# henriChevreux/distillation_trajectories

Measured on AMD Instinct MI355X. Metric: trajectory-timesteps/sec (B×T U-Net fwd) at 16×16 T=50, higher is better.
Workload: dtype f32 (fp32-accurate; convolutions: exact 3-plane bf16 operand split on bf16 MFMA with fp32 accumulate, or native fp32 MFMA, chosen per layer)

## Files before the change

### distillation_trajectories_amd/_hip.py

```python
import ctypes
import os
from ctypes import (POINTER, c_char_p, c_double, c_float, c_int, c_int32, c_int64, c_longlong, c_size_t, c_uint8,
                    c_void_p)

_LIB = None
LIB_PATH = os.path.join(os.path.dirname(os.path.abspath(__file__)), "csrc", "libdt_hip.so")

COND_NONE, COND_ZERO, COND_ONE = 0, 1, 2
RULE_ENGINE, RULE_PSAMPLE, RULE_MANAGER = 0, 1, 2
PREC_FP32, PREC_SPLIT_BF16, PREC_AUTO = 0, 1, 2
KIND_FP32 = 0
KIND_NAMES = {KIND_FP32: "fp32", 1: "split-bf16", 3: "split-bf16-strip", 4: "split-bf16-strip32", 5: "split-bf16-stripk"}
BT_COUNT, GT_COUNT, N_BLOCKS = 16, 9, 8
ABI_VERSION = 5


class HipLibraryError(RuntimeError):
    pass


class UNetDesc(ctypes.Structure):
    _fields_ = [("channels", c_int32), ("dims", c_int32 * 4), ("temb_dim", c_int32)]


SIGNATURES = {
    "dt_abi_version": (c_int, []),
    "dt_status_string": (c_char_p, [c_int]),
    "dt_unet_create": (c_int, [POINTER(UNetDesc), POINTER(c_void_p), POINTER(c_void_p), c_void_p, POINTER(c_void_p)]),
    "dt_unet_destroy": (None, [c_void_p]),
    "dt_unet_time_bias_stride": (c_int, [c_void_p]),
    "dt_unet_time_bias": (c_int, [c_void_p, c_void_p, c_void_p, c_void_p, c_int, c_void_p, c_void_p]),
    "dt_unet_workspace_bytes": (c_size_t, [c_void_p, c_int, c_int, c_int]),
    "dt_unet_forward": (c_int, [c_void_p, c_void_p, c_int, c_int, c_int, c_int, c_void_p, c_int, c_void_p,
                                c_void_p, c_size_t, c_void_p]),
    "dt_unet_autotune": (c_int, [c_void_p, c_int, c_int, c_int, c_void_p, c_size_t, c_void_p]),
    "dt_unet_conv_choice": (c_int, [c_void_p, c_int, c_int, c_int, c_int, c_int, POINTER(c_int), POINTER(c_int),
                                    POINTER(c_int), POINTER(c_int), POINTER(c_int)]),
    "dt_unet_set_conv_choice": (c_int, [c_void_p] + [c_int] * 10),
    "dt_unet_declare_shape": (c_int, [c_void_p] + [c_int] * 5),
    "dt_unet_set_precision": (c_int, [c_void_p, c_int]),
    "dt_unet_set_head_fusion": (c_int, [c_void_p, c_int]),
    "dt_unet_set_fused": (c_int, [c_void_p, c_int]),
    "dt_unet_fused_active": (c_int, [c_void_p, c_int, c_int]),
    "dt_unet_time_conv": (c_int, [c_void_p, c_int, c_int, c_int, c_int, c_int, c_int, c_int, c_int, c_int, c_int, c_int,
                                  c_void_p, c_size_t, c_void_p, POINTER(c_float), POINTER(c_double)]),
# ... 94 lines not shown
```

### distillation_trajectories_amd/csrc/build.py

```python
import os
import shutil
import subprocess
import sys

HERE = os.path.dirname(os.path.abspath(__file__))
SOURCES = ["dt_conv.hip", "dt_conv_bf16.hip", "dt_conv_strip.hip", "dt_layers.hip", "dt_update.hip", "dt_metrics.hip", "dt_fused.hip", "dt_unet.hip"]
HEADERS = ["dt_internal.h", "dt_conv_epilogue.h", "dt_update_math.h", "dt_fused.h", os.path.join("..", "..", "include", "dt_hip.h"),
           os.path.join("..", "..", "include", "dt_hip_noise.h")]
LIB = os.path.join(HERE, "libdt_hip.so")
ARCH = "gfx950"


def hipcc_path():
    for cand in (os.environ.get("HIPCC"), "/opt/rocm/bin/hipcc", shutil.which("hipcc")):
        if cand and os.path.exists(cand):
            return cand
    raise RuntimeError("hipcc not found (looked at $HIPCC, /opt/rocm/bin/hipcc, PATH)")


OBJ_DIR = os.path.join(HERE, "_build")
FLAGS = [f"--offload-arch={ARCH}", "-O3", "-std=c++17", "-fPIC", "-Wall", "-Wno-unused-function"]


def _newer(target, deps):
    if not os.path.exists(target):
        return True
    t = os.path.getmtime(target)
    return any(os.path.getmtime(d) > t for d in deps)


def is_stale():
    deps = [os.path.join(HERE, f) for f in SOURCES + HEADERS] + [os.path.abspath(__file__)]
    return _newer(LIB, deps)


TOOLS_MARK = os.path.join(OBJ_DIR, "tools_build")


def build(force=False, verbose=False, tools=False):
# ... 79 lines not shown
```

### distillation_trajectories_amd/csrc/dt_conv.hip

```cpp
#include "dt_conv_epilogue.h"

namespace dt {

template <int BM, int BN>
__global__ __launch_bounds__(256, 4) void conv_gemm_kernel(const ConvParams p) {
  constexpr int WN = 2;
  constexpr int MI = BM / 64, NI = BN / 64;
  constexpr int A_PER = BM / 64, B_PER = BN / 64;
  constexpr int STAGE = (BM + BN) * 16;
  constexpr int LDS_FLOATS = 2 * STAGE > epilogue_stage_floats<BN>() ? 2 * STAGE : epilogue_stage_floats<BN>();
  __shared__ __attribute__((aligned(16))) float lds[LDS_FLOATS];

  const int tid = threadIdx.x, lane = tid & 63, wave = tid >> 6;
  const int wm = wave / WN, wn = wave % WN;
  const int half = lane >> 5, l31 = lane & 31;
  const int m0 = blockIdx.x * BM, n0 = blockIdx.y * BN;
  const int HW = p.H * p.W;
  const int CC = p.cin_p >> 4;

  int a_off[A_PER], a_off2[A_PER], a_y[A_PER], a_x[A_PER];
  bool a_ok[A_PER];
  int a_lds[A_PER];
#pragma unroll
  for (int j = 0; j < A_PER; ++j) {
// ... 69 lines not shown
#pragma unroll
        for (int i = 0; i < 4; ++i)
#pragma unroll
          for (int mi = 0; mi < MI; ++mi)
#pragma unroll
            for (int ni = 0; ni < NI; ++ni) {
              acc[mi][ni] = __builtin_amdgcn_mfma_f32_32x32x2f32(fa[mi][i], fb[ni][i], acc[mi][ni], 0, 0, 0);
            }
      }
    }
    if (more) {
      float *A = lds + ((it + 1) & 1) * STAGE, *B = A + BM * 16;
#pragma unroll
      for (int j = 0; j < A_PER; ++j) *reinterpret_cast<f32x4 *>(A + a_lds[j]) = ra[j];
#pragma unroll
      for (int j = 0; j < B_PER; ++j) *reinterpret_cast<f32x4 *>(B + (tid + j * 256) * 4) = rb[j];
    }
    __syncthreads();
  }

  conv_epilogue<MI, NI>(p, acc, lds, m0, n0, wm, wn, half, l31);
}

int launch_splitk_epilogue(const ConvParams &p, hipStream_t s);

int launch_conv(const ConvParams &p, hipStream_t s) {
  if (!p.in || !p.w || !p.scale || !p.shift || !p.out) return DT_E_NULL;
  if (p.cin_p % 16 || p.cout_p % 16 || p.n_p % kNPad || p.M <= 0) return DT_E_SHAPE;
  if ((long long)p.M * p.cin_p >= (1ll << 31) || (long long)p.M * p.cout_p * (p.n_dup > 1 ? p.n_dup : 1) >= (1ll << 31)) return DT_E_SHAPE;
  if (const int st = conv_admissible(p)) return st;
  const bool tall_m = p.bm == 128, wide_n = p.bn == 128;
  dim3 grid((p.M + p.bm - 1) / p.bm, p.n_p / p.bn, p.splits);
  const double flops = 2.0 * p.M * (double)p.cout_real * ((double)p.cin_real * p.ksize * p.ksize + (p.in2 ? p.cin2_real : 0));
  if (is_strip(p.kind)) {
    ProfileScope prof(p.kind == KIND_STRIPK ? (tall_m ? KC_CONVS_K128x64 : (wide_n ? KC_CONVS_K64x128 : KC_CONVS_K64x64)) : p.bm == 256 ? KC_CONVS_256x64 : tall_m ? (wide_n ? KC_CONVS_128x128 : KC_CONVS_128x64) : (wide_n ? KC_CONVS_64x128 : KC_CONVS_64x64),
                      flops, 4.0 * p.M * ((double)p.cin_real + p.cout_real), s);
    const int st = launch_conv_strip(p, s);
    if (st) return st;
  } else if (p.kind == KIND_BF16) {
    ProfileScope prof(tall_m ? (wide_n ? KC_CONVB_128x128 : KC_CONVB_128x64) : (wide_n ? KC_CONVB_64x128 : KC_CONVB_64x64),
                      flops, 4.0 * p.M * ((double)p.cin_real + p.cout_real), s);
    const int st = launch_conv_bf16x6(p, p.bm, p.bn, s);
    if (st) return st;
  } else {
    ProfileScope prof(tall_m ? (wide_n ? KC_CONV_128x128 : KC_CONV_128x64) : (wide_n ? KC_CONV_64x128 : KC_CONV_64x64),
                      flops, 4.0 * p.M * ((double)p.cin_real + p.cout_real), s);
    if (tall_m && wide_n) conv_gemm_kernel<128, 128><<<grid, 256, 0, s>>>(p);
    else if (tall_m) conv_gemm_kernel<128, 64><<<grid, 256, 0, s>>>(p);
    else if (wide_n) conv_gemm_kernel<64, 128><<<grid, 256, 0, s>>>(p);
    else conv_gemm_kernel<64, 64><<<grid, 256, 0, s>>>(p);
    DT_LAUNCH_CHECK();
  }
  if (p.splits > 1) return launch_splitk_epilogue(p, s);
  return DT_OK;
}


int strip_kc(int kind, int bm, int bn) { return kind == KIND_STRIPK ? (bm == 64 && bn == 64 ? 4 : 2) : (kind == KIND_STRIP2 ? 2 : 1); }

size_t strip_lds_bytes(int W, int bm, int bn, int kind) {
  const int kc = strip_kc(kind, bm, bn);
  const int R = bm + 2 * strip_halo(W, bm);
  const size_t loop = (size_t)kc * ((size_t)3 * (((R + 7) & ~7) + 8) * 16 + (kind == KIND_STRIPK ? 0 : (size_t)2 * 3 * bn * 16)) * sizeof(__bf16);
  const size_t stage = (size_t)(bm == 256 || (kind == KIND_STRIPK && bn == 64) ? 128 : 64) * (bn + 4) * sizeof(float);
  return loop > stage ? loop : stage;
}

bool strip_reaches(int W) { return W + 1 <= 64 && strip_lds_bytes(W, 64, 64, KIND_STRIP) <= strip_lds_limit(KIND_STRIP); }

static bool kind_has_tile(int kind, int bm, int bn) {
  if (kind < KIND_FP32 || kind > KIND_STRIPK || kind == 2) return false;
  if ((bm != 64 && bm != 128 && !(bm == 256 && bn == 64 && is_strip(kind))) || (bn != 64 && bn != 128)) return false;
  return !(kind == KIND_STRIPK && (bm > 128 || (bm == 128 && bn == 128)));
}

bool conv_choice_valid(const ConvChoice &c, int slot, int n_p) {
  if (!kind_has_tile(c.kind, c.bm, c.bn) || n_p % c.bn) return false;
  if (c.splits < 1 || c.splits > 9 || c.splits == 5 || c.splits == 6 || c.splits == 7) return false;
  return !c.fuse || (slot == 2 && c.splits == 1);
}

static ConvChoice heuristic_choice(int M, int n_p, int taps) {
  ConvChoice c{};
  c.bn = n_p % 128 == 0 ? 128 : 64;
  const long long blocks128 = (long long)((M + 127) / 128) * (n_p / c.bn);
  c.bm = blocks128 >= 512 ? 128 : 64;
  const long long blocks = (long long)((M + c.bm - 1) / c.bm) * (n_p / c.bn);
  c.splits = 1;
  if (taps == 9 && M <= kSplitMaxRows && blocks < 384) c.splits = blocks * 3 >= 384 ? 3 : 9;
  c.fuse = c.splits == 1;
  return c;
}

ConvChoice resolve_conv_choice(const ConvLayer &L, const ConvChoice *req, int precision) {
  ConvChoice c = req ? *req : heuristic_choice(L.M, L.n_p, L.splittable ? L.taps : 1);
  const int cc = L.cin_p >> 4;
  if (!req) {
    c.kind = precision == DT_PREC_FP32 ? KIND_FP32 : KIND_BF16;
    if (c.kind == KIND_BF16 && L.taps == 9 && strip_reaches(L.W)) {
      c.kind = KIND_STRIP;
      c.splits = c.splits == 9 ? (cc % 8 == 0 ? 8 : (cc % 4 == 0 ? 4 : 1)) : (c.splits == 3 ? (cc % 4 == 0 ? 4 : (cc % 2 == 0 ? 2 : 1)) : 1);
    }
  }
  if (c.kind == 2) c.kind = KIND_BF16;
  if (is_strip(c.kind) && (L.taps != 9 || !strip_reaches(L.W))) c.kind = KIND_BF16;
  if (c.kind == KIND_STRIPK && (c.bm > 128 || (c.bm == 128 && c.bn == 128))) c.kind = KIND_STRIP2;
  if (c.bm == 256 && !is_strip(c.kind)) c.bm = 128;
  if (!L.splittable) c.splits = 1;
  if (is_strip(c.kind) ? !chunks_fit(cc, pack_chunks(L.cin_p), c.splits * strip_kc(c.kind, c.bm, c.bn)) : (L.taps * cc) % c.splits != 0)
    c.splits = 1;
  c.fuse = L.foldable && c.fuse && c.splits == 1;
  return c;
}

int conv_admissible(const ConvParams &p) {
  const int cc = p.cin_p >> 4;
  if (!kind_has_tile(p.kind, p.bm, p.bn) || p.n_p % p.bn) return DT_E_ARG;
  if (p.splits < 1 || (p.splits > 1 && !p.slab)) return DT_E_ARG;
  if (p.ccw < cc || (p.in2 && p.ccw2 < (p.cin2_p >> 4))) return DT_E_ARG;
  if (p.in2 && (p.splits != 1 || !p.w2 || !p.bias2 || p.cin2_p % 16)) return DT_E_ARG;
  if (!is_strip(p.kind)) return (p.tap_hi - p.tap_lo) * cc % p.splits ? DT_E_ARG : DT_OK;
  const int kc = strip_kc(p.kind, p.bm, p.bn);
  if (p.ksize != 3 || p.tap_lo != 0 || p.tap_hi != 9 || !chunks_fit(cc, p.ccw, p.splits * kc)) return DT_E_ARG;
  if (kc == 4 && p.W + 1 > 32) return DT_E_SHAPE;
  if (p.in2 && !chunks_fit(p.cin2_p >> 4, p.ccw2, kc)) return DT_E_ARG;
  if (p.W + 1 > 64) return DT_E_SHAPE;
  return strip_lds_bytes(p.W, p.bm, p.bn, p.kind) <= strip_lds_limit(p.kind) ? DT_OK : DT_E_SHAPE;
}

template <int S>
__device__ inline float4 splitk_finish(const ConvParams &p, unsigned m, int n, size_t slab_stride) {
  const size_t o = (size_t)m * p.cout_p + n;
  float4 a;
  if (S > 0) {
    float4 part[S > 0 ? S : 1];
#pragma unroll
    for (int z = 0; z < S; ++z) part[z] = *reinterpret_cast<const float4 *>(p.slab + z * slab_stride + o);
    a = part[0];
#pragma unroll
    for (int z = 1; z < S; ++z) { a.x += part[z].x; a.y += part[z].y; a.z += part[z].z; a.w += part[z].w; }
  } else {
    a = *reinterpret_cast<const float4 *>(p.slab + o);
    for (int z = 1; z < p.splits; ++z) {
      const float4 b = *reinterpret_cast<const float4 *>(p.slab + z * slab_stride + o);
      a.x += b.x; a.y += b.y; a.z += b.z; a.w += b.w;
    }
  }
  const float4 sc = *reinterpret_cast<const float4 *>(p.scale + n), sh = *reinterpret_cast<const float4 *>(p.shift + n);
  float4 v = make_float4(a.x * sc.x + sh.x, a.y * sc.y + sh.y, a.z * sc.z + sh.z, a.w * sc.w + sh.w);
  if (p.relu) { v.x = fmaxf(v.x, 0.f); v.y = fmaxf(v.y, 0.f); v.z = fmaxf(v.z, 0.f); v.w = fmaxf(v.w, 0.f); }
  if (p.tb) {
    const float4 t = *reinterpret_cast<const float4 *>(p.tb + (size_t)(m / (unsigned)p.m_per_tb) * p.tb_stride + n);
    v.x += t.x; v.y += t.y; v.z += t.z; v.w += t.w;
// ... 137 lines not shown
```

### distillation_trajectories_amd/csrc/dt_conv_epilogue.h

```cpp
#pragma once
#include "dt_internal.h"

namespace dt {

typedef float f32x16 __attribute__((ext_vector_type(16)));
typedef float f32x4 __attribute__((ext_vector_type(4)));

typedef __bf16 bf16x8 __attribute__((ext_vector_type(8)));
typedef __bf16 bf16x2 __attribute__((ext_vector_type(2)));
typedef unsigned u32x4 __attribute__((ext_vector_type(4)));

__device__ inline float bf16_to_f32(__bf16 v) { return (float)v; }

__device__ inline void split8(const f32x4 lo, const f32x4 hi, bf16x8 &p1, bf16x8 &p2, bf16x8 &p3) {
#pragma unroll
  for (int i = 0; i < 8; ++i) {
    const float a = i < 4 ? lo[i] : hi[i - 4];
    const __bf16 a1 = (__bf16)a;
    const float r1 = a - (float)a1;
    const __bf16 a2 = (__bf16)r1;
    const float r2 = r1 - (float)a2;
    p1[i] = a1; p2[i] = a2; p3[i] = (__bf16)r2;
  }
}

template <int BN, int WM = 2>
constexpr int epilogue_stage_floats() { return WM * 32 * (BN + 4); }

template <int MI, int NI, int WM = 2, int WK = 1>
__device__ inline void conv_epilogue(const ConvParams &p, f32x16 (&acc)[MI][NI], float *stage, int m0, int n0, int wm, int wn,
                                     int half, int l31, int wk = 0) {
  constexpr int BN = NI * 32 * (4 / (WM * WK)), P = BN + 4, C4 = BN / 4, U = WM * C4 / 8;
  constexpr int COPY = WM * 32 * P;
  const int tid = threadIdx.x;
  const int HW = p.H * p.W;
  const bool pow2 = (p.W & (p.W - 1)) == 0 && (HW & (HW - 1)) == 0;
  const int w_sh = 31 - __builtin_clz(p.W), hw_sh = 31 - __builtin_clz(HW);
  auto div_hw = [&](int m) { return pow2 ? m >> hw_sh : m / HW; };
  auto div_w = [&](int r) { return pow2 ? r >> w_sh : r / p.W; };
  const bool slab_mode = p.splits > 1;
  const size_t slab_stride = (size_t)p.M * p.cout_p;
  const int c4 = tid % C4, row0 = tid / C4;
  const int n = n0 + c4 * 4;
  const bool n_ok = n < p.cout_p;
  const int nn = n_ok ? n : 0;
  auto unit = [&](int k) __attribute__((always_inline)) {
    const float *src = stage + (row0 + k * (256 / C4)) * P + c4 * 4;
    f32x4 v = *reinterpret_cast<const f32x4 *>(src);
#pragma unroll
    for (int c = 1; c < WK; ++c) v += *reinterpret_cast<const f32x4 *>(src + c * COPY);
    return v;
  };
  auto unit_row = [&](int mi, int k) { const int row = row0 + k * (256 / C4); return m0 + (row >> 5) * (MI * 32) + mi * 32 + (row & 31); };
  auto to_stage = [&](int mi) __attribute__((always_inline)) {
    __syncthreads();
#pragma unroll
    for (int ni = 0; ni < NI; ++ni)
#pragma unroll
      for (int r = 0; r < 16; ++r) {
        const int L = 4 * half + (r & 3) + 8 * (r >> 2);
        stage[wk * COPY + (wm * 32 + L) * P + wn * (NI * 32) + ni * 32 + l31] = acc[mi][ni][r];
      }
    __syncthreads();
  };

  if (slab_mode) {
    float *slab = p.slab + (size_t)blockIdx.z * slab_stride;
#pragma unroll
    for (int mi = 0; mi < MI; ++mi) {
      to_stage(mi);
#pragma unroll
      for (int k = 0; k < U; ++k) {
        const int m = unit_row(mi, k);
        if (n_ok && m < p.M)
          *reinterpret_cast<f32x4 *>(slab + (size_t)m * p.cout_p + n) = unit(k);
      }
    }
    return;
  }

  auto pool_pass = [&](int mi, float *pool_out, const float *src, int n_src, int src_pitch, size_t out_pitch) __attribute__((always_inline)) {
    __syncthreads();
    const int Wo = p.W >> 1;
    for (int q0 = tid; q0 < n_src * WM * 8 * C4; q0 += 256) {
      const int pass = q0 / (WM * 8 * C4), q = q0 - pass * (WM * 8 * C4);
      const int pp = q / C4, qc = q % C4, j = pp & 7;
// ... 218 lines not shown
```

### distillation_trajectories_amd/csrc/dt_internal.h

```cpp
#pragma once
#include <hip/hip_runtime.h>
#include <stddef.h>
#include <stdint.h>

#include "../../include/dt_hip.h"

#define DT_HIP_TRY(expr)                         \
  do {                                           \
    hipError_t _e = (expr);                      \
    if (_e != hipSuccess) return (int)_e;        \
  } while (0)
#define DT_LAUNCH_CHECK()                        \
  do {                                           \
    hipError_t _e = hipGetLastError();           \
    if (_e != hipSuccess) return (int)_e;        \
  } while (0)

namespace dt {

enum KernelClass {
  KC_CONV_128x128 = 0, KC_CONV_128x64, KC_CONV_64x128, KC_CONV_64x64,
  KC_CONVB_128x128, KC_CONVB_128x64, KC_CONVB_64x128, KC_CONVB_64x64,
  KC_CONVS_128x128, KC_CONVS_128x64, KC_CONVS_64x128, KC_CONVS_64x64, KC_CONVS_256x64, KC_CONVS_K128x64, KC_CONVS_K64x64, KC_CONVS_K64x128,
  KC_SPLITK_EPILOGUE, KC_FIRST_CONV, KC_POOL, KC_UPCAT, KC_HEAD, KC_HEAD_UP, KC_TIME_BIAS, KC_UPDATE, KC_METRICS,
  KC_WASSERSTEIN, KC_RESAMPLE, KC_FUSED, KC_PAIR_METRICS,
  KC_COUNT
};
struct ProfileScope {
  ProfileScope(int cls, double flops, double bytes, hipStream_t s);
  ~ProfileScope();
  int slot;
  hipStream_t stream;
  void *end_event;
};

__device__ inline void bilinear_src(int dst, int in, int out, int &i0, int &i1, float &l0, float &l1) {
#pragma clang fp contract(off)
  const float scale = out > 1 ? (float)(in - 1) / (float)(out - 1) : 0.f;
  const float src = scale * (float)dst;
  i0 = (int)src;
  i1 = i0 + (i0 < in - 1 ? 1 : 0);
  l1 = src - (float)i0;
  l0 = 1.f - l1;
}
__device__ inline float bilinear_blend(float v00, float v01, float v10, float v11, float wy0, float wy1, float wx0, float wx1) {
  const float top = fmaf(wx1, v01, wx0 * v00), bot = fmaf(wx1, v11, wx0 * v10);
  return fmaf(wy1, bot, wy0 * top);
}

constexpr int kChanPad = 16;
constexpr int kNPad = 64;
constexpr int kBlocks = 8;
constexpr int kChunkPad = 4;

inline int round_up(int v, int m) { return (v + m - 1) / m * m; }
inline bool chunks_fit(int cc, int ccw, int div) { return div >= 1 && round_up(cc, div) <= ccw; }
inline int pack_chunks(int cin_p) { return round_up(cin_p, 16 * kChunkPad) >> 4; }

enum ConvKind {
  KIND_FP32 = 0,
  KIND_BF16 = 1,
  KIND_STRIP = 3,
  KIND_STRIP2 = 4,
  KIND_STRIPK = 5,
};
inline bool is_strip(int kind) { return kind >= KIND_STRIP; }

__host__ __device__ inline int strip_halo(int W, int bm) { return bm % W == 0 ? W : W + 1; }

struct ConvParams {
  const float *in;
  const float *w;
  const float *scale;
  const float *shift;
  const float *tb;
  const float *add;
  float *out;
  int M, H, W;
  int cin_p, cout_p, n_p;
  int cin_real, cout_real;
  int ksize;
  int tap_lo, tap_hi;
  int relu;
  int tb_stride;
  int m_per_tb;
  int splits;
  float *slab;
  int bm, bn;
  int kind;
  const float *x3;
  const float *w3;
  int x3_hw, x3_imgs, x3_c;
  const float *in2;
  const float *w2;
  const float *bias2;
  int cin2_p, cin2_real;
  float *pool_out;
  const float *in_b, *in2_b;
  int cc_a, b_stride;
  const float *head_w, *head_b;
  float *head_out;
  int head_c, head_cin;
  const float *tbc;
  int n_dup, dup_rows;
  int dup_skip;
  int skip_out;
  int dup_stage2;
  int ccw, ccw2;
  int ablate;
};

int launch_conv(const ConvParams &p, hipStream_t s);
int launch_conv_bf16x6(const ConvParams &p, int bm, int bn, hipStream_t s);
int launch_conv_strip(const ConvParams &p, hipStream_t s);
int launch_pack_conv_bf16x3(const float *w_oihw, void *wp, int cout, int cin, int ksize, int cin_p, int cin_w, int n_p,
                            int split_c, int split_cp, hipStream_t s);
constexpr int kSplitMaxRows = 32768;

struct ConvChoice { int bm, bn, splits, kind, fuse; };
struct ConvLayer {
  int M, W;
  int n_p, cin_p;
  int taps;
  bool splittable;
  bool foldable;
};
int strip_kc(int kind, int bm, int bn);
size_t strip_lds_bytes(int W, int bm, int bn, int kind);
inline size_t strip_lds_limit(int kind) { return kind == KIND_STRIP ? 65536u : 98304u; }
bool strip_reaches(int W);
bool conv_choice_valid(const ConvChoice &c, int slot, int n_p);
ConvChoice resolve_conv_choice(const ConvLayer &L, const ConvChoice *req, int precision);
int conv_admissible(const ConvParams &p);

int launch_pack_conv(const float *w_oihw, float *wp, int cout, int cin, int ksize, int cin_p, int n_p,
                     int split_c, int split_cp, hipStream_t s);
int launch_fold_bn(const float *conv_b, const float *g, const float *b, const float *mean, const float *var,
                   float *scale, float *shift, int cout, int n_p, hipStream_t s);
int launch_pack_linear_rows(const float *w, const float *b, float *wp, float *bp, int out, int in, int out_p,
                            hipStream_t s);

int launch_first_conv(const float *x, const float *wf, const float *scale, const float *shift, const float *tb, int tb_stride,
                      int tb_div, float *out, int B, int n_pass, int C, int H, int W, int cout, int cout_p, hipStream_t s);
int launch_pack_first_conv(const float *w_oihw, float *wf, int cout, int C, int cout_p, hipStream_t s);
int launch_pack_tap_major(const float *w_oihw, float *w2t, int cout, int cin, int cp, hipStream_t s);
int launch_maxpool(const float *in, float *out, int Bt, int H, int W, int cp, hipStream_t s);
int launch_upcat(const float *lo, const float *skip, float *out, int Bt, int h, int w, int c1p, int c2p,
                 hipStream_t s);
int launch_head(const float *lo, const float *w, const float *bias, float *lowres, int Bt, int h, int w_, int cp, int C, int c_real,
                hipStream_t s);
int launch_head_upsample(const float *lowres, float *eps, int Bt, int h, int w_, int C, hipStream_t s);
int launch_pack_res3(const float *w, const float *b, float *w3, int cout, int C, int n_p, hipStream_t s);

struct TembWeights {
  const float *freqs;
  const float *w1, *b1;
  const float *wc0, *bc0;
  const float *wc2, *bc2;
  const float *wt, *bt;
  int D, half, tb_stride;
  int tb_cols;
  const float *w2t;
  int c0p;
};
int launch_time_bias(const TembWeights &tw, const int32_t *t, const float *cond, const uint8_t *present, int rows,
                     float *out, hipStream_t s);
// ... 3 lines not shown
```

### distillation_trajectories_amd/csrc/dt_unet.hip

```cpp
#include <algorithm>
#include <atomic>
#include <cstdio>
#include <cstdlib>
#include <cstring>
#include <mutex>
#include <new>
#include <vector>

#include "dt_fused.h"
#include "dt_internal.h"
#include "../../include/dt_hip_noise.h"

namespace dt {
int launch_cfg_update(int rule, const float *x, const float *eu, const float *ec, const float *z,
                      const int32_t *z_row, long long z_shift, const float coef[4], int has_noise, const float *w,
                      float w_scalar, float *out, int B, int E, hipStream_t s);
int launch_cfg_update_lowres(int rule, const float *x, const float *lowres_u, const float *lowres_c, const float *z,
                             const int32_t *z_row, long long z_shift, const float coef[4], int has_noise, const float *w,
                             float w_scalar, float *out, int B, int C, int H, int W, int b_single, hipStream_t s);
int launch_traj_metrics(const float *X, const float *Y, int nT, int nS, int B, int E, double *out, hipStream_t s);
int launch_wasserstein(const float *X, const float *Y, int n, int B, int E, const int32_t *index,
                       const int32_t *index_row, int n_idx, double *out, hipStream_t s);
int launch_resampled_distance(const float *L, const float *S, int n_long, int n_short, int B, int E, double *out,
                              hipStream_t s);
// ... 1 lines not shown
int launch_pair_stats(const float *X, const float *Y, int n, int B, int E, double *out, hipStream_t s);
int launch_sample_mean(const float *traj, int n, int B, int E, float *out, hipStream_t s);
int launch_resize_bilinear(const float *in, float *out, int planes, int h, int w, int H, int W, hipStream_t s);
int launch_q_sample(const float *x0, const float *z, const float *coef, int n_groups, int B, int E, float *out, hipStream_t s);
}

using namespace dt;

namespace {
struct ProfRecord { hipEvent_t a, b; int cls; double flops, bytes; };
struct Profiler {
  std::mutex mu;
  std::atomic<bool> on{false};
  std::vector<ProfRecord> rec;
  std::vector<hipEvent_t> pool;
  size_t used = 0;
  hipEvent_t get() {
    if (used == pool.size()) {
      hipEvent_t e;
      if (hipEventCreate(&e) != hipSuccess) return nullptr;
      pool.push_back(e);
    }
    return pool[used++];
  }
} g_prof;
const char *kClassName[KC_COUNT] = {
    "conv_gemm_kernel<128,128>", "conv_gemm_kernel<128,64>", "conv_gemm_kernel<64,128>", "conv_gemm_kernel<64,64>",
    "conv_gemm_bf16x6_kernel<128,128>", "conv_gemm_bf16x6_kernel<128,64>", "conv_gemm_bf16x6_kernel<64,128>",
    "conv_gemm_bf16x6_kernel<64,64>",
    "conv_strip_bf16x6_kernel<128,128>", "conv_strip_bf16x6_kernel<128,64>", "conv_strip_bf16x6_kernel<64,128>",
    "conv_strip_bf16x6_kernel<64,64>", "conv_strip_bf16x6_kernel<256,64>", "conv_strip_bf16x6_kernel<128,64,K2>",
    "conv_strip_bf16x6_kernel<64,64,K4>", "conv_strip_bf16x6_kernel<64,128,K2>", "splitk_epilogue_kernel", "first_conv_kernel", "maxpool_kernel", "upcat_kernel", "head_kernel", "head_upsample_kernel",
    "time_bias_kernel", "cfg_update_kernel", "traj_metrics_kernel", "wasserstein_kernel", "resampled_distance_kernel",
    "unet_fused_kernel", "pair_metrics_kernel"};
}

namespace dt {
ProfileScope::ProfileScope(int cls, double flops, double bytes, hipStream_t s) : slot(-1), stream(s), end_event(nullptr) {
  if (!g_prof.on.load(std::memory_order_relaxed)) return;
  hipEvent_t a;
  {
    std::lock_guard<std::mutex> lock(g_prof.mu);
    if (!g_prof.on.load(std::memory_order_relaxed)) return;
    a = g_prof.get();
    hipEvent_t b = g_prof.get();
    if (!a || !b) return;
    g_prof.rec.push_back(ProfRecord{a, b, cls, flops, bytes});
    slot = (int)g_prof.rec.size() - 1;
    end_event = b;
  }
  (void)hipEventRecord(a, s);
}
ProfileScope::~ProfileScope() {
  if (slot < 0) return;
  (void)hipEventRecord((hipEvent_t)end_event, stream);
}
}

struct BlockW {
  int cin, cout;
  int cin_p, cout_p, n_p;
  int split_c, split_cp;
  int cin_w, cout_w;
  bool has_res;
  float *w1, *w2, *wr;
  float *w1b, *w2b, *wrb;
  float *s1, *h1, *s2, *h2, *sr, *hr;
// ... 101 lines not shown
void shape_images(const dt_unet *u, int Bt, int H, int W, int &imgs, int &single) {
  {
    std::lock_guard<std::mutex> lock(u->shape_mu);
    for (const ShapeInfo &si : u->shapes)
      if (si.Bt == Bt && si.H == H && si.W == W) { imgs = si.imgs; single = si.single; return; }
  }
  imgs = Bt % 2 == 0 ? Bt / 2 : Bt;
  single = 0;
}

void note_shape(const dt_unet *u, int Bt, int H, int W, int imgs, int single) {
  std::lock_guard<std::mutex> lock(u->shape_mu);
  for (ShapeInfo &si : u->shapes)
    if (si.Bt == Bt && si.H == H && si.W == W) { si.imgs = imgs; si.single = single; return; }
  u->shapes.push_back(ShapeInfo{Bt, H, W, imgs, single});
}

struct ResolvedForward {
  int Bt, H, W, imgs, single;
  bool shared_enc1;
  ConvChoice c[kBlocks][3];
  bool pool_fused[kBlocks];
  bool concat_in_place[kBlocks];
  bool head_fused;
};

bool has_launch(const dt_unet *u, int j, int slot) { return slot == 2 || (j > 0 && (slot == 1 || u->blk[j].has_res)); }

ConvLayer conv_layer(const dt_unet *u, const ResolvedForward &f, int j, int slot) {
  const BlockW &k = u->blk[j];
  const int h = f.H / kDiv[j], w = f.W / kDiv[j];
  const int M = (j == 0 && f.shared_enc1 ? f.imgs : f.Bt) * h * w;
  const int taps = slot == 0 || (h == 1 && w == 1) ? 1 : 9;
  return ConvLayer{M, w, k.n_p, slot == 2 ? k.cout_p : k.cin_p, taps, j > 0 && M <= kSplitMaxRows, slot == 2 && j > 0 && k.has_res};
}

ResolvedForward resolve_forward(const dt_unet *u, int Bt, int H, int W, int imgs, int single, const TunedShape *tuned) {
  ResolvedForward f{};
  f.Bt = Bt; f.H = H; f.W = W; f.imgs = imgs; f.single = single;
  f.shared_enc1 = u->share_enc1 && (Bt + single) % imgs == 0;
  for (int j = 0; j < kBlocks; ++j)
    for (int slot = 0; slot < 3; ++slot)
      if (has_launch(u, j, slot)) f.c[j][slot] = resolve_conv_choice(conv_layer(u, f, j, slot), tuned ? &tuned->c[j][slot] : nullptr, u->precision);
  for (int j = 0; j < kBlocks; ++j) {
    const ConvChoice &c2 = f.c[j][2];
    const int h = H / kDiv[j], w = W / kDiv[j];
    f.pool_fused[j] = j <= 3 && h % 2 == 0 && w % 2 == 0 && (c2.splits > 1 || (w <= 16 && (w & (w - 1)) == 0));
    f.concat_in_place[j] = j >= 5 && u->blk[j].has_res && is_strip(f.c[j][1].kind) && is_strip(c2.kind) && c2.fuse;
  }
  const ConvChoice &last = f.c[kBlocks - 1][2];
  f.head_fused = u->head_fusion && last.splits == 1 && u->blk[kBlocks - 1].n_p == last.bn && u->desc.channels <= 3;
  return f;
}

ConvParams bind_conv(const dt_unet *u, const ResolvedForward &f, int j, int slot, const ConvChoice &c, const float *in, float *ws,
                     const Plan &pl, const float *tb, int tb_div) {
  const BlockW &k = u->blk[j];
  const ConvLayer L = conv_layer(u, f, j, slot);
  const int h = pl.H[j], w = pl.W[j];
  ConvParams p{};
  p.M = L.M; p.H = h; p.W = w;
  p.cin_p = L.cin_p; p.cout_p = k.cout_p; p.n_p = k.n_p;
  p.cin_real = slot == 2 ? k.cout : k.cin; p.cout_real = k.cout;
  p.tb_stride = u->tb_stride; p.m_per_tb = h * w * tb_div;
  p.slab = ws + pl.slab;
  p.in = slot == 2 ? ws + pl.h[j] : in;
  p.ksize = slot == 0 ? 1 : 3;
  p.tap_lo = slot > 0 && L.taps == 1 ? 4 : 0; p.tap_hi = p.tap_lo + L.taps;
  p.relu = slot > 0;
  if (slot == 0) {
    p.scale = k.sr; p.shift = k.hr; p.out = ws + pl.r[j];
  } else if (slot == 1) {
    p.scale = k.s1; p.shift = k.h1; p.tb = tb + k.tb_off; p.out = ws + pl.h[j];
  } else {
    p.scale = k.s2; p.shift = k.h2; p.out = ws + pl.o[j];
    if (f.pool_fused[j]) p.pool_out = ws + pl.pool[j];
    if (j == 0) {
      p.x3 = in; p.w3 = k.w3; p.x3_hw = h * w; p.x3_imgs = f.imgs; p.x3_c = u->desc.channels;
      if (f.shared_enc1) {
        p.n_dup = (f.Bt + f.single) / f.imgs; p.dup_rows = p.M; p.dup_skip = f.single * h * w; p.tbc = tb + u->tb_cols;
        p.skip_out = u->head_fusion && p.pool_out ? 1 : 0;
      }
    } else {
      p.add = k.has_res ? ws + pl.r[j] : in;
// ... 348 lines not shown
  {
    const ConvParams wp = bind_conv(h, f, 1, 1, f.c[1][1], ws + pl.pool[0], ws, pl, tb, batch_total);
    for (int rep = 0; rep < 200 && st == DT_OK; ++rep) st = launch_conv(wp, s);
    if (hipStreamSynchronize(s) != hipSuccess) st = (int)hipGetLastError();
  }
  for (int j = 0; j < kBlocks && st == DT_OK; ++j) {
    const float *in = j == 0 ? ws + pl.h[0] : (j <= 4 ? ws + pl.pool[j - 1] : ws + pl.cat[j - 5]);
    float skip_ms = 0.f;
    for (int slot = 0; slot < 3 && st == DT_OK; ++slot) {
      if (!has_launch(h, j, slot)) continue;
      ConvChoice best = f.c[j][slot];
      best.fuse = 0;
      const ConvLayer L = conv_layer(h, f, j, slot);
      float best_ms = 1e30f;
      auto measure = [&](const ConvParams &q, int reps) -> float {
        int lst = launch_conv(q, s);
        if (lst == DT_E_SHAPE || lst == DT_E_ARG) return -1.f;
        if (lst != DT_OK) { st = lst; return -1.f; }
        (void)hipEventRecord(e0, s);
        for (int rep = 0; rep < reps && lst == DT_OK; ++rep) lst = launch_conv(q, s);
        (void)hipEventRecord(e1, s);
        if (hipEventSynchronize(e1) != hipSuccess) lst = (int)hipGetLastError();
        if (lst != DT_OK) { st = lst; return -1.f; }
        float ms = 0.f;
        (void)hipEventElapsedTime(&ms, e0, e1);
        return ms / reps;
      };
      struct Cand { ConvChoice c; ConvParams q; float cost; };
      std::vector<Cand> cands;
      auto cost_of = [&](float ms, const ConvChoice &c) {
        return (ms + (c.fuse ? 0.f : (L.foldable ? skip_ms : 0.f))) * (c.splits > 1 ? kSplitMargin : 1.0f);
      };
      const bool strip_ok = L.taps == 9 && strip_reaches(L.W);
      for (const int kind : {KIND_FP32, KIND_BF16, KIND_STRIP, KIND_STRIP2, KIND_STRIPK}) {
        if (h->precision == DT_PREC_FP32 ? kind != KIND_FP32 : kind == KIND_FP32) continue;
        if (is_strip(kind) ? !strip_ok : (kind == KIND_BF16 && strip_ok)) continue;
        for (int bm = 64; bm <= 256; bm *= 2)
          for (int bn = 64; bn <= 128; bn += 64) {
            if (j == kBlocks - 1 && slot == 2 && h->head_fusion && h->desc.channels <= 3 && L.n_p <= 128 && bn != L.n_p) continue;
            const long long tiles = (long long)((L.M + bm - 1) / bm) * (L.n_p / bn);
            for (int sp = 1; sp <= (L.splittable ? 9 : 1); sp *= ((is_strip(kind) || L.taps != 9) ? 2 : 3))
              for (int fuse = 0; fuse <= ((L.foldable && sp == 1) ? 1 : 0); ++fuse) {
                if (sp > 1 && tiles * (sp / 2) >= 1024) continue;
                const ConvChoice c{bm, bn, sp, kind, fuse};
                const ConvParams q = bind_conv(h, f, j, slot, c, in, ws, pl, tb, batch_total);
                if (conv_admissible(q) != DT_OK) continue;
                const float ms = measure(q, 3);
                if (ms < 0.f) continue;
                cands.push_back(Cand{c, q, cost_of(ms, c)});
              }
          }
      }
      if (!cands.empty() && st == DT_OK) {
        std::vector<size_t> top;
        for (size_t i = 0; i < cands.size(); ++i) top.push_back(i);
        std::stable_sort(top.begin(), top.end(), [&](size_t a, size_t b) { return cands[a].cost < cands[b].cost; });
        if (top.size() > 3) top.resize(3);
        std::sort(top.begin(), top.end());
        std::vector<float> fin(top.size(), 1e30f);
        for (int round = 0; round < 2 && st == DT_OK; ++round)
          for (size_t k = 0; k < top.size() && st == DT_OK; ++k) {
            const float ms = measure(cands[top[k]].q, 10);
            if (ms >= 0.f && ms < fin[k]) fin[k] = ms;
          }
        for (size_t k = 0; k < top.size(); ++k) {
          const float cost = cost_of(fin[k], cands[top[k]].c);
          if (cost < best_ms * 1.01f) { best_ms = cost < best_ms ? cost : best_ms; best = cands[top[k]].c; }
        }
      }
      t.c[j][slot] = best;
      if (slot == 0) skip_ms = best_ms;
    }
  }
  (void)hipEventDestroy(e0);
// ... 316 lines not shown
```

Measured before the change: 348,400.

## Add position-major split-bf16 conv kernel for small spatial layers

Adds a new convolution kernel in which each block handles one spatial position across a tile of images. It walks only the taps that are valid at that position, so padded taps at border pixels cost no loads or MFMAs. The autotuner now considers this kernel for 3x3 layers with at most 64 pixels, and strip-kernel choices at 2x2 resolution are silently redirected to it. The goal is to remove wasted halo and padding work in the deep low-resolution layers. In exchange it adds extra dispatch rules, and pooled or head-fused epilogues are disallowed unless split-K is used.

After: 352,700, median of 6. 1.2% higher.

```diff
diff --git a/distillation_trajectories_amd/_hip.py b/distillation_trajectories_amd/_hip.py
--- a/distillation_trajectories_amd/_hip.py
+++ b/distillation_trajectories_amd/_hip.py
@@ -10,7 +10,7 @@
 RULE_ENGINE, RULE_PSAMPLE, RULE_MANAGER = 0, 1, 2
 PREC_FP32, PREC_SPLIT_BF16, PREC_AUTO = 0, 1, 2
 KIND_FP32 = 0
-KIND_NAMES = {KIND_FP32: "fp32", 1: "split-bf16", 3: "split-bf16-strip", 4: "split-bf16-strip32", 5: "split-bf16-stripk"}
+KIND_NAMES = {KIND_FP32: "fp32", 1: "split-bf16", 3: "split-bf16-strip", 4: "split-bf16-strip32", 5: "split-bf16-stripk", 6: "split-bf16-pos"}
 BT_COUNT, GT_COUNT, N_BLOCKS = 16, 9, 8
 ABI_VERSION = 5
 
diff --git a/distillation_trajectories_amd/csrc/build.py b/distillation_trajectories_amd/csrc/build.py
--- a/distillation_trajectories_amd/csrc/build.py
+++ b/distillation_trajectories_amd/csrc/build.py
@@ -4,7 +4,7 @@
 import sys
 
 HERE = os.path.dirname(os.path.abspath(__file__))
-SOURCES = ["dt_conv.hip", "dt_conv_bf16.hip", "dt_conv_strip.hip", "dt_layers.hip", "dt_update.hip", "dt_metrics.hip", "dt_fused.hip", "dt_unet.hip"]
+SOURCES = ["dt_conv.hip", "dt_conv_bf16.hip", "dt_conv_strip.hip", "dt_conv_pos.hip", "dt_layers.hip", "dt_update.hip", "dt_metrics.hip", "dt_fused.hip", "dt_unet.hip"]
 HEADERS = ["dt_internal.h", "dt_conv_epilogue.h", "dt_update_math.h", "dt_fused.h", os.path.join("..", "..", "include", "dt_hip.h"),
            os.path.join("..", "..", "include", "dt_hip_noise.h")]
 LIB = os.path.join(HERE, "libdt_hip.so")
diff --git a/distillation_trajectories_amd/csrc/dt_conv.hip b/distillation_trajectories_amd/csrc/dt_conv.hip
--- a/distillation_trajectories_amd/csrc/dt_conv.hip
+++ b/distillation_trajectories_amd/csrc/dt_conv.hip
@@ -125,7 +125,14 @@
   const bool tall_m = p.bm == 128, wide_n = p.bn == 128;
   dim3 grid((p.M + p.bm - 1) / p.bm, p.n_p / p.bn, p.splits);
   const double flops = 2.0 * p.M * (double)p.cout_real * ((double)p.cin_real * p.ksize * p.ksize + (p.in2 ? p.cin2_real : 0));
-  if (is_strip(p.kind)) {
+  if (p.kind == KIND_POS || strip_runs_as_position(p)) {
+    ConvParams q = p;
+    q.kind = KIND_POS;
+    ProfileScope prof(tall_m ? (wide_n ? KC_CONVP_128x128 : KC_CONVP_128x64) : (wide_n ? KC_CONVP_64x128 : KC_CONVP_64x64),
+                      flops, 4.0 * p.M * ((double)p.cin_real + p.cout_real), s);
+    const int st = launch_conv_pos(q, s);
+    if (st) return st;
+  } else if (is_strip(p.kind)) {
     ProfileScope prof(p.kind == KIND_STRIPK ? (tall_m ? KC_CONVS_K128x64 : (wide_n ? KC_CONVS_K64x128 : KC_CONVS_K64x64)) : p.bm == 256 ? KC_CONVS_256x64 : tall_m ? (wide_n ? KC_CONVS_128x128 : KC_CONVS_128x64) : (wide_n ? KC_CONVS_64x128 : KC_CONVS_64x64),
                       flops, 4.0 * p.M * ((double)p.cin_real + p.cout_real), s);
     const int st = launch_conv_strip(p, s);
@@ -162,9 +169,9 @@
 bool strip_reaches(int W) { return W + 1 <= 64 && strip_lds_bytes(W, 64, 64, KIND_STRIP) <= strip_lds_limit(KIND_STRIP); }
 
 static bool kind_has_tile(int kind, int bm, int bn) {
-  if (kind < KIND_FP32 || kind > KIND_STRIPK || kind == 2) return false;
+  if (kind < KIND_FP32 || kind > KIND_POS || kind == 2) return false;
   if ((bm != 64 && bm != 128 && !(bm == 256 && bn == 64 && is_strip(kind))) || (bn != 64 && bn != 128)) return false;
-  return !(kind == KIND_STRIPK && (bm > 128 || (bm == 128 && bn == 128)));
+  return !((kind == KIND_STRIPK || kind == KIND_POS) && (bm > 128 || (bm == 128 && bn == 128)));
 }
 
 bool conv_choice_valid(const ConvChoice &c, int slot, int n_p) {
@@ -196,14 +203,26 @@
     }
   }
   if (c.kind == 2) c.kind = KIND_BF16;
+  if (c.kind == KIND_POS && (L.taps != 9 || (L.pooled && (c.splits == 1 || !L.splittable))))
+    c.kind = strip_reaches(L.W) && L.taps == 9 ? KIND_STRIP2 : KIND_BF16;
   if (is_strip(c.kind) && (L.taps != 9 || !strip_reaches(L.W))) c.kind = KIND_BF16;
   if (c.kind == KIND_STRIPK && (c.bm > 128 || (c.bm == 128 && c.bn == 128))) c.kind = KIND_STRIP2;
   if (c.bm == 256 && !is_strip(c.kind)) c.bm = 128;
   if (!L.splittable) c.splits = 1;
-  if (is_strip(c.kind) ? !chunks_fit(cc, pack_chunks(L.cin_p), c.splits * strip_kc(c.kind, c.bm, c.bn)) : (L.taps * cc) % c.splits != 0)
+  const int kc = is_strip(c.kind) ? strip_kc(c.kind, c.bm, c.bn) : (c.kind == KIND_POS ? kPosKC : 0);
+  if (kc ? !chunks_fit(cc, pack_chunks(L.cin_p), c.splits * kc) : (L.taps * cc) % c.splits != 0) {
     c.splits = 1;
+    if (c.kind == KIND_POS && L.pooled) c.kind = strip_reaches(L.W) ? KIND_STRIP2 : KIND_BF16;
+  }
   c.fuse = L.foldable && c.fuse && c.splits == 1;
   return c;
+}
+
+bool strip_runs_as_position(const ConvParams &p) {
+  if (!is_strip(p.kind) || p.H != 2 || p.W != 2) return false;
+  ConvParams q = p;
+  q.kind = KIND_POS;
+  return conv_admissible(q) == DT_OK;
 }
 
 int conv_admissible(const ConvParams &p) {
@@ -212,6 +231,12 @@
   if (p.splits < 1 || (p.splits > 1 && !p.slab)) return DT_E_ARG;
   if (p.ccw < cc || (p.in2 && p.ccw2 < (p.cin2_p >> 4))) return DT_E_ARG;
   if (p.in2 && (p.splits != 1 || !p.w2 || !p.bias2 || p.cin2_p % 16)) return DT_E_ARG;
+  if (p.kind == KIND_POS) {
+    if (p.ksize != 3 || p.tap_lo != 0 || p.tap_hi != 9 || p.H < 2 || p.W < 2 || p.M % (p.H * p.W)) return DT_E_ARG;
+    if (!chunks_fit(cc, p.ccw, p.splits * kPosKC) || (p.in2 && !chunks_fit(p.cin2_p >> 4, p.ccw2, kPosKC))) return DT_E_ARG;
+    if (p.splits == 1 && (p.pool_out || p.n_dup || p.head_out || p.x3)) return DT_E_ARG;
+    return DT_OK;
+  }
   if (!is_strip(p.kind)) return (p.tap_hi - p.tap_lo) * cc % p.splits ? DT_E_ARG : DT_OK;
   const int kc = strip_kc(p.kind, p.bm, p.bn);
   if (p.ksize != 3 || p.tap_lo != 0 || p.tap_hi != 9 || !chunks_fit(cc, p.ccw, p.splits * kc)) return DT_E_ARG;
diff --git a/distillation_trajectories_amd/csrc/dt_conv_epilogue.h b/distillation_trajectories_amd/csrc/dt_conv_epilogue.h
--- a/distillation_trajectories_amd/csrc/dt_conv_epilogue.h
+++ b/distillation_trajectories_amd/csrc/dt_conv_epilogue.h
@@ -27,9 +27,9 @@
 template <int BN, int WM = 2>
 constexpr int epilogue_stage_floats() { return WM * 32 * (BN + 4); }
 
-template <int MI, int NI, int WM = 2, int WK = 1>
+template <int MI, int NI, int WM = 2, int WK = 1, bool POS = false>
 __device__ inline void conv_epilogue(const ConvParams &p, f32x16 (&acc)[MI][NI], float *stage, int m0, int n0, int wm, int wn,
-                                     int half, int l31, int wk = 0) {
+                                     int half, int l31, int wk = 0, int pos = 0) {
   constexpr int BN = NI * 32 * (4 / (WM * WK)), P = BN + 4, C4 = BN / 4, U = WM * C4 / 8;
   constexpr int COPY = WM * 32 * P;
   const int tid = threadIdx.x;
@@ -51,7 +51,10 @@
     for (int c = 1; c < WK; ++c) v += *reinterpret_cast<const f32x4 *>(src + c * COPY);
     return v;
   };
-  auto unit_row = [&](int mi, int k) { const int row = row0 + k * (256 / C4); return m0 + (row >> 5) * (MI * 32) + mi * 32 + (row & 31); };
+  auto unit_row = [&](int mi, int k) {
+    const int row = row0 + k * (256 / C4), r = (row >> 5) * (MI * 32) + mi * 32 + (row & 31);
+    return POS ? (m0 + r) * HW + pos : m0 + r;
+  };
   auto to_stage = [&](int mi) __attribute__((always_inline)) {
     __syncthreads();
 #pragma unroll
diff --git a/distillation_trajectories_amd/csrc/dt_conv_pos.hip b/distillation_trajectories_amd/csrc/dt_conv_pos.hip
--- /dev/null
+++ b/distillation_trajectories_amd/csrc/dt_conv_pos.hip
@@ -0,0 +1,186 @@
+#include "dt_conv_epilogue.h"
+
+namespace dt {
+
+__device__ inline void pos_of_rank(int k, int H, int W, int &y, int &x) {
+  const int iw = W - 2, ih = H - 2;
+  if (k < ih * iw) { y = 1 + k / iw; x = 1 + k % iw; return; }
+  k -= ih * iw;
+  if (k < 2 * iw) { y = k < iw ? 0 : H - 1; x = 1 + k % iw; return; }
+  k -= 2 * iw;
+  if (k < 2 * ih) { x = k < ih ? 0 : W - 1; y = 1 + k % ih; return; }
+  k -= 2 * ih;
+  y = (k >> 1) ? H - 1 : 0;
+  x = (k & 1) ? W - 1 : 0;
+}
+
+template <int BM, int BN, int WM>
+__global__ __launch_bounds__(256, 2) void conv_pos_bf16x6_kernel(const ConvParams p) {
+  constexpr int WN = 4 / WM, KC = 2;
+  constexpr int MI = BM / (32 * WM), NI = BN / (32 * WN);
+  static_assert(MI * 32 * WM == BM && NI * 32 * WN == BN, "wave layout");
+  constexpr int PLANE_B = BN * 16, STAGE_B = 3 * PLANE_B;
+  constexpr int LDS_B = 2 * KC * STAGE_B * 2, LDS_E = epilogue_stage_floats<BN, WM>() * 4;
+  __shared__ __attribute__((aligned(16))) unsigned char lds_raw[LDS_B > LDS_E ? LDS_B : LDS_E];
+  __bf16 *Bs = reinterpret_cast<__bf16 *>(lds_raw);
+
+  const int tid = threadIdx.x, lane = tid & 63;
+  const int wave = __builtin_amdgcn_readfirstlane(tid >> 6);
+  const int wm = wave / WN, wn = wave % WN;
+  const int half = lane >> 5, l31 = lane & 31;
+  const int HW = p.H * p.W;
+  const int B = p.M / HW;
+  const int nib = (B + BM - 1) / BM, nnb = p.n_p / BN;
+  const int ib = blockIdx.x % nib, rest = blockIdx.x / nib;
+  const int nb = rest % nnb, rank = rest / nnb;
+  int py, px;
+  pos_of_rank(rank, p.H, p.W, py, px);
+  const int pos = py * p.W + px;
+  const int img0 = ib * BM, n0 = nb * BN;
+  unsigned tmask = 0;
+#pragma unroll
+  for (int t = 0; t < 9; ++t) {
+    const int yy = py + t / 3 - 1, xx = px + t % 3 - 1;
+    if (yy >= 0 && yy < p.H && xx >= 0 && xx < p.W) tmask |= 1u << t;
+  }
+
+  bool a_ok[MI];
+  int a_pix[MI];
+#pragma unroll
+  for (int mi = 0; mi < MI; ++mi) {
+    const int img = img0 + wm * (MI * 32) + mi * 32 + l31;
+    a_ok[mi] = img < B;
+    a_pix[mi] = a_ok[mi] ? img * HW + pos : 0;
+  }
+  const bool b_thread = tid < BN * 2;
+  const size_t w_plane = (size_t)p.n_p * 16;
+  const __bf16 *wbase = reinterpret_cast<const __bf16 *>(p.w) + (size_t)n0 * 16 + tid * 8;
+  const __bf16 *wbase2 = reinterpret_cast<const __bf16 *>(p.w2) + (size_t)n0 * 16 + tid * 8;
+  int b_frag[NI];
+#pragma unroll
+  for (int ni = 0; ni < NI; ++ni) {
+    const int row = wn * (NI * 32) + ni * 32 + l31;
+    b_frag[ni] = row * 16 + ((half ^ ((row >> 3) & 1)) << 3);
+  }
+
+  f32x16 acc[MI][NI];
+#pragma unroll
+  for (int mi = 0; mi < MI; ++mi)
+#pragma unroll
+    for (int ni = 0; ni < NI; ++ni)
+#pragma unroll
+      for (int r = 0; r < 16; ++r) acc[mi][ni][r] = 0.f;
+
+  const int CC = p.cin_p >> 4, CC2 = p.cin2_p >> 4;
+  const int n_main = (CC + p.splits * KC - 1) / (p.splits * KC);
+  const int cc0 = blockIdx.z * n_main * KC;
+  const int n_skip = p.in2 ? (CC2 + KC - 1) / KC : 0;
+  const int n_main_steps = __builtin_popcount(tmask) * n_main;
+  const int n_steps = n_main_steps + n_skip;
+  struct WalkPos { unsigned rem; int tap, g; };
+  auto advance = [&](WalkPos &w) __attribute__((always_inline)) {
+    if (w.rem && ++w.g == n_main) {
+      w.g = 0;
+      w.rem &= w.rem - 1;
+      w.tap = w.rem ? __builtin_ctz(w.rem) : 0;
+    } else if (!w.rem) {
+      ++w.g;
+    }
+  };
+
+  f32x4 ga0[KC][MI][2], ga1[KC][MI][2];
+  auto load_a = [&](f32x4 (&g)[KC][MI][2], const WalkPos &w) __attribute__((always_inline)) {
+    const int shift = (w.tap / 3 - 1) * p.W + (w.tap % 3 - 1);
+#pragma unroll
+    for (int kk = 0; kk < KC; ++kk)
+#pragma unroll
+      for (int mi = 0; mi < MI; ++mi) {
+        g[kk][mi][0] = f32x4{0.f, 0.f, 0.f, 0.f}; g[kk][mi][1] = g[kk][mi][0];
+        const float *src = nullptr;
+        if (w.rem) {
+          const int cc = cc0 + w.g * KC + kk;
+          const size_t pix = (size_t)(a_pix[mi] + shift);
+          if (a_ok[mi] && cc < CC)
+            src = (p.in_b && cc >= p.cc_a) ? p.in_b + pix * p.b_stride + (cc - p.cc_a) * 16 + half * 8 : p.in + pix * p.cin_p + cc * 16 + half * 8;
+        } else {
+          const int c2 = w.g * KC + kk;
+          const size_t pix = (size_t)a_pix[mi];
+          if (a_ok[mi] && c2 < CC2)
+            src = (p.in2_b && c2 >= p.cc_a) ? p.in2_b + pix * p.b_stride + (c2 - p.cc_a) * 16 + half * 8 : p.in2 + pix * p.cin2_p + c2 * 16 + half * 8;
+        }
+        if (src) {
+          g[kk][mi][0] = *reinterpret_cast<const f32x4 *>(src);
+          g[kk][mi][1] = *reinterpret_cast<const f32x4 *>(src + 4);
+        }
+      }
+  };
+  u32x4 rb0[KC * 3], rb1[KC * 3];
+  auto load_b = [&](u32x4 (&rb)[KC * 3], const WalkPos &w) __attribute__((always_inline)) {
+    if (!b_thread) return;
+    const __bf16 *wt = w.rem ? wbase + (size_t)(w.tap * p.ccw + cc0 + w.g * KC) * 3 * w_plane : wbase2 + (size_t)(w.g * KC) * 3 * w_plane;
+#pragma unroll
+    for (int i = 0; i < KC * 3; ++i) rb[i] = *reinterpret_cast<const u32x4 *>(wt + i * w_plane);
+  };
+  auto write_b = [&](const u32x4 (&rb)[KC * 3], int stage) __attribute__((always_inline)) {
+    if (!b_thread) return;
+    __bf16 *Bt = Bs + stage * KC * STAGE_B + tid * 8;
+#pragma unroll
+    for (int i = 0; i < KC * 3; ++i) *reinterpret_cast<u32x4 *>(Bt + i * PLANE_B) = rb[i];
+  };
+
+  const unsigned first_tap = tmask ? __builtin_ctz(tmask) : 0;
+  WalkPos wa{tmask, (int)first_tap, 0}, wb = wa;
+  if (n_steps > 0) { load_a(ga0, wa); advance(wa); load_b(rb0, wb); advance(wb); write_b(rb0, 0); }
+  if (n_steps > 1) { load_a(ga1, wa); advance(wa); load_b(rb1, wb); advance(wb); }
+  __syncthreads();
+
+  auto step = [&](f32x4 (&g)[KC][MI][2], u32x4 (&rb_this)[KC * 3], u32x4 (&rb_next)[KC * 3], int s) __attribute__((always_inline)) {
+    if (s == n_main_steps && p.in2) conv_midpoint<MI, NI>(p, acc, n0, wn, l31);
+    if (s + 2 < n_steps) { load_b(rb_this, wb); advance(wb); }
+    const __bf16 *Bst = Bs + (s & 1) * KC * STAGE_B;
+#pragma unroll
+    for (int kk = 0; kk < KC; ++kk) {
+      bf16x8 fb[NI][3];
+#pragma unroll
+      for (int ni = 0; ni < NI; ++ni)
+#pragma unroll
+        for (int pl = 0; pl < 3; ++pl) fb[ni][pl] = *reinterpret_cast<const bf16x8 *>(Bst + kk * STAGE_B + pl * PLANE_B + b_frag[ni]);
+#pragma unroll
+      for (int mi = 0; mi < MI; ++mi) {
+        bf16x8 fa[3];
+        split8(g[kk][mi][0], g[kk][mi][1], fa[0], fa[1], fa[2]);
+#pragma unroll
+        for (int ni = 0; ni < NI; ++ni) {
+          f32x16 c = acc[mi][ni];
+          c = __builtin_amdgcn_mfma_f32_32x32x16_bf16(fa[2], fb[ni][0], c, 0, 0, 0);
+          c = __builtin_amdgcn_mfma_f32_32x32x16_bf16(fa[1], fb[ni][1], c, 0, 0, 0);
+          c = __builtin_amdgcn_mfma_f32_32x32x16_bf16(fa[0], fb[ni][2], c, 0, 0, 0);
+          c = __builtin_amdgcn_mfma_f32_32x32x16_bf16(fa[1], fb[ni][0], c, 0, 0, 0);
+          c = __builtin_amdgcn_mfma_f32_32x32x16_bf16(fa[0], fb[ni][1], c, 0, 0, 0);
+          c = __builtin_amdgcn_mfma_f32_32x32x16_bf16(fa[0], fb[ni][0], c, 0, 0, 0);
+          acc[mi][ni] = c;
+        }
+      }
+    }
+    if (s + 2 < n_steps) { load_a(g, wa); advance(wa); }
+    if (s + 1 < n_steps) write_b(rb_next, (s + 1) & 1);
+    __syncthreads();
+  };
+  for (int s = 0; s < n_steps; s += 2) {
+    step(ga0, rb0, rb1, s);
+    if (s + 1 < n_steps) step(ga1, rb1, rb0, s + 1);
+  }
+  conv_epilogue<MI, NI, WM, 1, true>(p, acc, reinterpret_cast<float *>(lds_raw), img0, n0, wm, wn, half, l31, 0, pos);
+}
+
+int launch_conv_pos(const ConvParams &p, hipStream_t s) {
+  const int HW = p.H * p.W, B = p.M / HW;
+  dim3 grid(HW * ((B + p.bm - 1) / p.bm) * (p.n_p / p.bn), 1, p.splits);
+  if (p.bm == 128) conv_pos_bf16x6_kernel<128, 64, 4><<<grid, 256, 0, s>>>(p);
+  else if (p.bn == 128) conv_pos_bf16x6_kernel<64, 128, 2><<<grid, 256, 0, s>>>(p);
+  else conv_pos_bf16x6_kernel<64, 64, 2><<<grid, 256, 0, s>>>(p);
+  DT_LAUNCH_CHECK();
+  return DT_OK;
+}
+
+}
diff --git a/distillation_trajectories_amd/csrc/dt_internal.h b/distillation_trajectories_amd/csrc/dt_internal.h
--- a/distillation_trajectories_amd/csrc/dt_internal.h
+++ b/distillation_trajectories_amd/csrc/dt_internal.h
@@ -24,6 +24,7 @@
   KC_CONVS_128x128, KC_CONVS_128x64, KC_CONVS_64x128, KC_CONVS_64x64, KC_CONVS_256x64, KC_CONVS_K128x64, KC_CONVS_K64x64, KC_CONVS_K64x128,
   KC_SPLITK_EPILOGUE, KC_FIRST_CONV, KC_POOL, KC_UPCAT, KC_HEAD, KC_HEAD_UP, KC_TIME_BIAS, KC_UPDATE, KC_METRICS,
   KC_WASSERSTEIN, KC_RESAMPLE, KC_FUSED, KC_PAIR_METRICS,
+  KC_CONVP_128x128, KC_CONVP_128x64, KC_CONVP_64x128, KC_CONVP_64x64,
   KC_COUNT
 };
 struct ProfileScope {
@@ -63,8 +64,11 @@
   KIND_STRIP = 3,
   KIND_STRIP2 = 4,
   KIND_STRIPK = 5,
+  KIND_POS = 6,
 };
-inline bool is_strip(int kind) { return kind >= KIND_STRIP; }
+inline bool is_strip(int kind) { return kind >= KIND_STRIP && kind <= KIND_STRIPK; }
+inline bool reads_concat_in_place(int kind) { return is_strip(kind) || kind == KIND_POS; }
+constexpr int kPosKC = 2;
 
 __host__ __device__ inline int strip_halo(int W, int bm) { return bm % W == 0 ? W : W + 1; }
 
@@ -113,17 +117,19 @@
 int launch_conv(const ConvParams &p, hipStream_t s);
 int launch_conv_bf16x6(const ConvParams &p, int bm, int bn, hipStream_t s);
 int launch_conv_strip(const ConvParams &p, hipStream_t s);
+int launch_conv_pos(const ConvParams &p, hipStream_t s);
 int launch_pack_conv_bf16x3(const float *w_oihw, void *wp, int cout, int cin, int ksize, int cin_p, int cin_w, int n_p,
                             int split_c, int split_cp, hipStream_t s);
 constexpr int kSplitMaxRows = 32768;
 
 struct ConvChoice { int bm, bn, splits, kind, fuse; };
 struct ConvLayer {
-  int M, W;
+  int M, H, W;
   int n_p, cin_p;
   int taps;
   bool splittable;
   bool foldable;
+  bool pooled;
 };
 int strip_kc(int kind, int bm, int bn);
 size_t strip_lds_bytes(int W, int bm, int bn, int kind);
@@ -132,6 +138,7 @@
 bool conv_choice_valid(const ConvChoice &c, int slot, int n_p);
 ConvChoice resolve_conv_choice(const ConvLayer &L, const ConvChoice *req, int precision);
 int conv_admissible(const ConvParams &p);
+bool strip_runs_as_position(const ConvParams &p);
 
 int launch_pack_conv(const float *w_oihw, float *wp, int cout, int cin, int ksize, int cin_p, int n_p,
                      int split_c, int split_cp, hipStream_t s);
diff --git a/distillation_trajectories_amd/csrc/dt_unet.hip b/distillation_trajectories_amd/csrc/dt_unet.hip
--- a/distillation_trajectories_amd/csrc/dt_unet.hip
+++ b/distillation_trajectories_amd/csrc/dt_unet.hip
@@ -57,7 +57,8 @@
     "conv_strip_bf16x6_kernel<64,64>", "conv_strip_bf16x6_kernel<256,64>", "conv_strip_bf16x6_kernel<128,64,K2>",
     "conv_strip_bf16x6_kernel<64,64,K4>", "conv_strip_bf16x6_kernel<64,128,K2>", "splitk_epilogue_kernel", "first_conv_kernel", "maxpool_kernel", "upcat_kernel", "head_kernel", "head_upsample_kernel",
     "time_bias_kernel", "cfg_update_kernel", "traj_metrics_kernel", "wasserstein_kernel", "resampled_distance_kernel",
-    "unet_fused_kernel", "pair_metrics_kernel"};
+    "unet_fused_kernel", "pair_metrics_kernel",
+    "conv_pos_bf16x6_kernel<128,128>", "conv_pos_bf16x6_kernel<128,64>", "conv_pos_bf16x6_kernel<64,128>", "conv_pos_bf16x6_kernel<64,64>"};
 }
 
 namespace dt {
@@ -225,7 +226,8 @@
   const int h = f.H / kDiv[j], w = f.W / kDiv[j];
   const int M = (j == 0 && f.shared_enc1 ? f.imgs : f.Bt) * h * w;
   const int taps = slot == 0 || (h == 1 && w == 1) ? 1 : 9;
-  return ConvLayer{M, w, k.n_p, slot == 2 ? k.cout_p : k.cin_p, taps, j > 0 && M <= kSplitMaxRows, slot == 2 && j > 0 && k.has_res};
+  return ConvLayer{M, h, w, k.n_p, slot == 2 ? k.cout_p : k.cin_p, taps, j > 0 && M <= kSplitMaxRows, slot == 2 && j > 0 && k.has_res,
+                   slot == 2 && j <= 3 && h % 2 == 0 && w % 2 == 0};
 }
 
 ResolvedForward resolve_forward(const dt_unet *u, int Bt, int H, int W, int imgs, int single, const TunedShape *tuned) {
@@ -239,10 +241,10 @@
     const ConvChoice &c2 = f.c[j][2];
     const int h = H / kDiv[j], w = W / kDiv[j];
     f.pool_fused[j] = j <= 3 && h % 2 == 0 && w % 2 == 0 && (c2.splits > 1 || (w <= 16 && (w & (w - 1)) == 0));
-    f.concat_in_place[j] = j >= 5 && u->blk[j].has_res && is_strip(f.c[j][1].kind) && is_strip(c2.kind) && c2.fuse;
+    f.concat_in_place[j] = j >= 5 && u->blk[j].has_res && reads_concat_in_place(f.c[j][1].kind) && reads_concat_in_place(c2.kind) && c2.fuse;
   }
   const ConvChoice &last = f.c[kBlocks - 1][2];
-  f.head_fused = u->head_fusion && last.splits == 1 && u->blk[kBlocks - 1].n_p == last.bn && u->desc.channels <= 3;
+  f.head_fused = u->head_fusion && last.splits == 1 && u->blk[kBlocks - 1].n_p == last.bn && u->desc.channels <= 3 && last.kind != KIND_POS;
   return f;
 }
 
@@ -657,14 +659,15 @@
         return (ms + (c.fuse ? 0.f : (L.foldable ? skip_ms : 0.f))) * (c.splits > 1 ? kSplitMargin : 1.0f);
       };
       const bool strip_ok = L.taps == 9 && strip_reaches(L.W);
-      for (const int kind : {KIND_FP32, KIND_BF16, KIND_STRIP, KIND_STRIP2, KIND_STRIPK}) {
+      for (const int kind : {KIND_FP32, KIND_BF16, KIND_STRIP, KIND_STRIP2, KIND_STRIPK, KIND_POS}) {
         if (h->precision == DT_PREC_FP32 ? kind != KIND_FP32 : kind == KIND_FP32) continue;
         if (is_strip(kind) ? !strip_ok : (kind == KIND_BF16 && strip_ok)) continue;
+        if (kind == KIND_POS && (L.taps != 9 || L.H * L.W > 64)) continue;
         for (int bm = 64; bm <= 256; bm *= 2)
           for (int bn = 64; bn <= 128; bn += 64) {
             if (j == kBlocks - 1 && slot == 2 && h->head_fusion && h->desc.channels <= 3 && L.n_p <= 128 && bn != L.n_p) continue;
             const long long tiles = (long long)((L.M + bm - 1) / bm) * (L.n_p / bn);
-            for (int sp = 1; sp <= (L.splittable ? 9 : 1); sp *= ((is_strip(kind) || L.taps != 9) ? 2 : 3))
+            for (int sp = 1; sp <= (L.splittable ? 9 : 1); sp *= ((is_strip(kind) || kind == KIND_POS || L.taps != 9) ? 2 : 3))
               for (int fuse = 0; fuse <= ((L.foldable && sp == 1) ? 1 : 0); ++fuse) {
                 if (sp > 1 && tiles * (sp / 2) >= 1024) continue;
                 const ConvChoice c{bm, bn, sp, kind, fuse};
```
